# mic-rud/Learned-Compression-of-Point-Cloud-Geometry-and-Attributes

Hardware: AMD Instinct MI355X
Metric: encode+decode Mpoints/sec (higher is better)
Workload: dtype f32

## Files before the change

include/pcc_hip.h:

```cpp
#ifndef PCC_HIP_H
#define PCC_HIP_H

#include <stdint.h>

#ifdef __cplusplus
extern "C" {
#endif

#define PCC_OK 0
#define PCC_ERR_ARG (-1)
#define PCC_ERR_HIP (-2)
#define PCC_ERR_UNSUPPORTED (-3)
#define PCC_ERR_DATA (-4)

#define PCC_ACT_NONE 0
#define PCC_ACT_RELU 1
#define PCC_ACT_LEAKY_RELU 2

int pcc_version(void);
const char* pcc_last_error(void);
int pcc_device_count(void);
int pcc_device_name(int dev, char* out, int out_len);

int64_t pcc_hash_capacity(int64_t n);
// ... 37 lines not shown
                   int32_t sign, int32_t* nbr, uint32_t* row_mask, int64_t* pair_count,
                   void* stream);

int pcc_pair_count(const uint32_t* row_mask, int64_t n_out, int64_t* pair_count, void* stream);

int64_t pcc_order_scratch_bytes(int64_t n);
int pcc_order_rows_by_mask(const uint32_t* row_mask, const int32_t* coords, int64_t n,
                           int32_t block_log2, int32_t tensor_stride, int32_t* order, uint32_t* group_mask32,
                           void* scratch, int64_t scratch_bytes, void* stream);
int pcc_permute_map_rows(const int32_t* nbr, const int32_t* order, int64_t n, int32_t K, int32_t* nbr_sorted, void* stream);

int64_t pcc_small_map_max(void);
int32_t pcc_small_paths(int32_t mask);
int pcc_small_kernel_map(const int32_t* out_coords, int64_t n_out, const uint64_t* in_keys, const int32_t* in_vals, int64_t in_cap,
                         int32_t ksize, int32_t step, int32_t sign, int32_t* nbr, uint32_t* row_mask, int32_t* order,
                         uint32_t* group_mask32, void* scratch, int64_t scratch_bytes, void* stream);

int64_t pcc_conv_packed_elems(int32_t K, int32_t cin, int32_t cout);
int pcc_conv_pack_weights(const float* w, int32_t K, int32_t cin, int32_t cout, float* w_packed,
                          void* stream);
int pcc_conv_fwd(const float* fin, int64_t n_in, int32_t cin, const float* w, const float* w_packed,
                 const float* bias, const int32_t* nbr, const int32_t* order,
                 const uint32_t* group_mask32, int32_t K, float* fout, int64_t n_out, int32_t cout,
                 int32_t act, const float* film, const float* residual, void* stream);

int64_t pcc_conv_small_max(int64_t workgroups);

int pcc_conv_kernel_name(int32_t mode, int64_t n_in, int32_t cin, int32_t cout, int64_t n_out, int32_t K, int32_t has_nbr,
                         char* buf, int32_t len);

int64_t pcc_conv_packed_elems_bf16(int32_t K, int32_t cin, int32_t cout);
int pcc_conv_pack_weights_bf16(const float* w, int32_t K, int32_t cin, int32_t cout, uint16_t* w_packed, void* stream);
int pcc_conv_fwd_bf16(const uint16_t* fin, int64_t n_in, int32_t cin, const uint16_t* w_packed, const float* bias,
                      const int32_t* nbr, const int32_t* order, const uint32_t* group_mask32, int32_t K, float* fout,
                      int64_t n_out, int32_t cout, int32_t act, const float* film, const float* residual, void* stream);

int pcc_epilogue_fwd(const float* c, const float* film, const float* residual, int64_t n, int32_t channels, int32_t act,
                     float* out, void* stream);
int pcc_epilogue_bwd(const float* dout, const float* c, const float* film, int64_t n, int32_t channels, int32_t act,
                     float* dc, float* dfilm, void* stream);

int64_t pcc_cast_colsum_scratch_elems(int32_t channels);
int pcc_cast_colsum(const float* x, int64_t n, int32_t channels, uint16_t* out_bf16, float* colsum, float* scratch,
                    int64_t scratch_elems, void* stream);

int64_t pcc_conv_packed_elems_x3(int32_t K, int32_t cin, int32_t cout);
int pcc_conv_pack_weights_x3(const float* w, int32_t K, int32_t cin, int32_t cout, uint16_t* w_packed, void* stream);
int pcc_conv_fwd_x3(const float* fin, int64_t n_in, int32_t cin, const uint16_t* w_packed, const float* bias,
                    const int32_t* nbr, const int32_t* order, const uint32_t* group_mask32, int32_t K, float* fout,
                    int64_t n_out, int32_t cout, int32_t act, const float* film, const float* residual, void* stream);

int pcc_im2col_thin(const float* fin, int32_t cin, const int32_t* nbr, int64_t n_out, int32_t K, float* out, int32_t k2,
                    void* stream);

int pcc_gather_sum_fwd(const float* scores, int32_t ld, const int32_t* nbr, int32_t K, int32_t cout,
                       const float* bias, float* out, int64_t n_out, int32_t act, void* stream);

int pcc_gather_rows(const float* src, int32_t c, const int32_t* idx, int64_t n, float* out,
                    int32_t accumulate, void* stream);

int pcc_scatter_rows(const float* src, int32_t c, const int32_t* idx, int64_t n, float* out,
                     void* stream);
int pcc_scatter_add_rows(const float* src, int32_t c, const int32_t* idx, int64_t n, float* out,
                         void* stream);

int pcc_compact_rows(const uint8_t* mask, int64_t n, const int32_t* coords, int32_t* out_coords,
                     const float* feats, int32_t c, float* out_feats, int32_t* new_index,
                     int32_t* scratch, int64_t* out_count, void* stream);

int64_t pcc_topk_state_elems(int32_t nbatch);
int pcc_topk_mask(const float* logits, int32_t ld, const int32_t* coords, int64_t n, int32_t nbatch,
                  const int32_t* k, uint8_t* mask, int32_t* state, void* stream);

int pcc_count_per_batch(const int32_t* coords, int64_t n, int32_t nbatch, int32_t* counts, void* stream);

int64_t pcc_sort_scratch_bytes(int64_t n);
int pcc_sort_coords(const int32_t* coords, int64_t n, int32_t* perm, void* scratch,
                    int64_t scratch_bytes, void* stream);

int pcc_kernel_map_transpose(const int32_t* nbr, int64_t n_out, int32_t K, int64_t n_in, int32_t* nbr_t,
                             uint32_t* row_mask_t, void* stream);
int64_t pcc_conv_wgrad_scratch_elems(int32_t K, int32_t cin, int32_t cout);
int pcc_conv_wgrad(const float* fin, int64_t n_in, int32_t cin, const float* dy, int64_t n_out, int32_t cout,
                   const int32_t* nbr, const int32_t* order, const uint32_t* group_mask32, int32_t K, float* dw,
                   float* scratch, int64_t scratch_elems, void* stream);
int pcc_conv_wgrad_kernel_name(int32_t bf16, int32_t K, int32_t cin, int32_t cout, int64_t n_out, char* buf, int32_t len,
                               int32_t* split, int32_t* partials);
int pcc_conv_wgrad_bf16(const uint16_t* fin, int64_t n_in, int32_t cin, const uint16_t* dy, int64_t n_out, int32_t cout,
                        const int32_t* nbr, const int32_t* order, const uint32_t* group_mask32, int32_t K, float* dw,
                        float* scratch, int64_t scratch_elems, void* stream);

int pcc_chconv(const float* x, int64_t n, int32_t c, const int32_t* coords, const uint64_t* keys, const int32_t* vals,
               int64_t cap, int32_t tensor_stride, int32_t ksize, const float* w, int32_t w_channels, int32_t flip,
               float* y, void* stream);

int64_t pcc_octree_scratch_bytes(int64_t n);
int pcc_octree_occupancy(const int32_t* coords, int64_t n, int32_t stride, const int32_t* origin,
                         int32_t depth, uint8_t* occupancy, int32_t* level_counts, void* scratch,
                         int64_t scratch_bytes, void* stream);
int pcc_octree_expand(const uint8_t* occupancy, const int64_t* level_counts, int32_t depth,
                      int32_t stride, const int32_t* origin, int32_t batch, int64_t n_points,
                      int32_t* coords_out, void* scratch, int64_t scratch_bytes, void* stream);

int pcc_nn_search(const int32_t* query, int64_t nq, const uint64_t* keys, const int32_t* vals, int64_t cap,
                  int32_t tensor_stride, const double* target_rgb, int32_t max_radius, int32_t* nn_idx, int64_t* nn_d2,
                  int32_t* tie_count, double* tie_rgb, void* stream);
// ... 92 lines not shown
```

learned-compression-of-point-cloud-geometry-and-attributes_amd/_build.py:

```python
import os
import subprocess

_HERE = os.path.dirname(os.path.abspath(__file__))
SO_PATH = os.path.join(_HERE, "libpcc_hip.so")

NO_SCRATCH = {
    "conv": ("conv_small_kernel", "conv_mfma_buf_kernel", "conv_mfma_kernel"),
    "rans_lanes": ("rans_lanes_encode_kernel", "rans_lanes_pack_kernel", "rans_lanes_decode_kernel"),
    "chconv": ("chconv_kernel",),
    "augment": ("jitter_partial_kernel", "jitter_mean_kernel", "jitter_apply_kernel", "first_rows_clear_kernel",
                "first_rows_insert_kernel", "first_rows_flag_kernel", "first_rows_finalize_kernel"),
    "normals": ("estimate_normals_kernel",),
    "voxelize": ("first_rows_clear_kernel", "first_rows_insert_kernel", "first_rows_flag_kernel", "first_rows_finalize_kernel",
                 "voxelize_accumulate_kernel"),
    "raht": ("raht_plan_kernel", "raht_step_kernel", "raht_fold_kernel"),
}


def build(force=False):
    args = ["make", "-s", "-C", os.path.join(_HERE, "csrc"), "-j4"]
    if force:
        subprocess.check_call(args + ["clean"])
    subprocess.check_call(args)
    for stem, kernels in NO_SCRATCH.items():
        check_kernel_resources(os.path.join(_HERE, "build", stem + ".resources.txt"), kernels)
    check_small_kernel_lds_reads()
    return SO_PATH


def check_small_kernel_lds_reads(obj=None):
    import glob
    import shutil
    objdump = "/opt/rocm/lib/llvm/bin/llvm-objdump"
    obj = obj or os.path.join(_HERE, "build", "conv.o")
    if not os.path.exists(objdump) or not os.path.exists(obj):
        raise RuntimeError(f"cannot lint conv_small_kernel: {objdump} or {obj} is missing")
    tmp = os.path.join(_HERE, "build", "_lint")
    shutil.rmtree(tmp, ignore_errors=True)
    os.makedirs(tmp)
    local = os.path.join(tmp, "conv.o")
    shutil.copy(obj, local)
    subprocess.run([objdump, "--offloading", local], check=True, capture_output=True, cwd=tmp)
    cos = [f for f in glob.glob(local + ".*") if "amdgcn" in f]
    if not cos:
        raise RuntimeError("cannot lint conv_small_kernel: no device code object in build/conv.o")
    dis = subprocess.run([objdump, "-d", cos[0]], check=True, capture_output=True, text=True).stdout
    shutil.rmtree(tmp, ignore_errors=True)
    return lint_lds_reads(dis)


def lint_lds_reads(dis, kernel="conv_small_kernel"):
    import re

    def regs(operand):
        m = re.fullmatch(r"v\[(\d+):(\d+)\]", operand)
        if m:
            return set(range(int(m.group(1)), int(m.group(2)) + 1))
        m = re.fullmatch(r"v(\d+)", operand)
        return {int(m.group(1))} if m else set()

# ... 64 lines not shown
```

learned-compression-of-point-cloud-geometry-and-attributes_amd/csrc/conv.hip:

```cpp
#include <stdlib.h>

#include <type_traits>

#include "common.h"

namespace pcc {

typedef float f32x2 __attribute__((ext_vector_type(2)));
typedef float f32x4 __attribute__((ext_vector_type(4)));
typedef __bf16 bf16x8 __attribute__((ext_vector_type(8)));

struct ConvArgs {
    const float* fin;
    const float* w;
    const float* wp;
    const float* bias;
    const int32_t* nbr;
    const int32_t* order;
    const uint32_t* gmask;
    float* fout;
    const float* film;
    const float* residual;
    int64_t n_in, n_out;
    int cin, cout, coutp, K, act;
// ... 768 lines not shown
        for (int j = 0; j < CPT; ++j) acc[j] = 0.0f;
        for (int k0 = 0; k0 < K; k0 += 9) {
            int idx[9];
#pragma unroll
            for (int u = 0; u < 9; ++u) idx[u] = (k0 + u < K) ? (a.nbr ? a.nbr[row * K + k0 + u] : (int)row) : -1;
            float in[9][CIN];
#pragma unroll
            for (int u = 0; u < 9; ++u) {
                const int64_t src = idx[u] >= 0 ? idx[u] : 0;
#pragma unroll
                for (int ci = 0; ci < CIN; ++ci) in[u][ci] = a.fin[src * CIN + ci];
            }
#pragma unroll
            for (int u = 0; u < 9; ++u) {
                if (idx[u] < 0) continue;
                const float* wk = smem + ((k0 + u) * CIN) * cout + co;
#pragma unroll
                for (int ci = 0; ci < CIN; ++ci)
#pragma unroll
                    for (int j = 0; j < CPT; ++j) acc[j] = fmaf(in[u][ci], wk[ci * cout + j], acc[j]);
            }
        }
#pragma unroll
        for (int j = 0; j < CPT; ++j) conv_store(a, row, co + j, acc[j], conv_bias(a, co + j));
    }
}

__global__ __launch_bounds__(256) void im2col_thin_kernel(const float* __restrict__ fin, int cin, const int32_t* __restrict__ nbr,
                                                          int64_t n_out, int K, float* __restrict__ out, int k2) {
    const int q = k2 >> 2;
    const int64_t total = n_out * q;
    const int kc = K * cin;
    for (int64_t e = (int64_t)blockIdx.x * 256 + threadIdx.x; e < total; e += (int64_t)gridDim.x * 256) {
        const int64_t row = e / q;
        const int c0 = (int)(e - row * q) * 4;
        f32x4 v;
#pragma unroll
        for (int s = 0; s < 4; ++s) {
            const int c = c0 + s;
            const int s8 = c & 7;
            const int logical = (c & ~7) + ((s8 & 3) << 1 | (s8 >> 2));
            float x = 0.0f;
            if (logical < kc) {
                const int k = logical / cin, ci = logical - k * cin;
                const int idx = nbr[row * K + k];
                if (idx >= 0) x = fin[(int64_t)idx * cin + ci];
            }
            v[s] = x;
        }
        *reinterpret_cast<f32x4*>(out + row * k2 + c0) = v;
    }
}

__global__ __launch_bounds__(256) void gather_sum_kernel(const float* __restrict__ scores, int ld,
                                                         const int32_t* __restrict__ nbr, int K, int cout,
                                                         const float* __restrict__ bias, float* __restrict__ out,
                                                         int64_t n_out, int act) {
    const int64_t total = n_out * cout;
    for (int64_t e = (int64_t)blockIdx.x * 256 + threadIdx.x; e < total; e += (int64_t)gridDim.x * 256) {
        const int64_t row = e / cout;
        const int c = (int)(e - row * cout);
        float acc = 0.0f;
        for (int k = 0; k < K; ++k) {
            const int idx = nbr[row * K + k];
            if (idx >= 0) acc += scores[(int64_t)idx * ld + k * cout + c];
        }
        out[e] = apply_act(acc + (bias ? bias[c] : 0.0f), act);
    }
}

template <int COUT>
__global__ __launch_bounds__(256) void gather_sum27_kernel(const float* __restrict__ scores, int ld,
                                                           const int32_t* __restrict__ nbr, const float* __restrict__ bias,
                                                           float* __restrict__ out, int64_t n_out, int act) {
    __shared__ __attribute__((aligned(16))) int32_t idx_s[256 * 27];
    const int64_t row0 = (int64_t)blockIdx.x * 256;
    const int64_t rows = (n_out - row0 < 256) ? (n_out - row0) : 256;
    const int64_t words = rows * 27;
    const int32_t* src = nbr + row0 * 27;
    for (int64_t w = 4 * (int64_t)threadIdx.x; w < words; w += 1024) {
        if (w + 4 <= words) {
            *reinterpret_cast<int4*>(idx_s + w) = *reinterpret_cast<const int4*>(src + w);
        } else {
            for (int64_t u = w; u < words; ++u) idx_s[u] = src[u];
        }
    }
    __syncthreads();
    if ((int64_t)threadIdx.x >= rows) return;
    const int32_t* mine = idx_s + threadIdx.x * 27;
    float acc[COUT];
#pragma unroll
    for (int c = 0; c < COUT; ++c) acc[c] = 0.0f;
#pragma unroll
    for (int k0 = 0; k0 < 27; k0 += 9) {
        int idx[9];
        float v[9][COUT];
#pragma unroll
        for (int u = 0; u < 9; ++u) idx[u] = mine[k0 + u];
#pragma unroll
        for (int u = 0; u < 9; ++u) {
            const float* sp = scores + (int64_t)(idx[u] >= 0 ? idx[u] : 0) * ld + (k0 + u) * COUT;
#pragma unroll
            for (int c = 0; c < COUT; ++c) v[u][c] = sp[c];
        }
#pragma unroll
        for (int u = 0; u < 9; ++u)
            if (idx[u] >= 0) {
#pragma unroll
                for (int c = 0; c < COUT; ++c) acc[c] += v[u][c];
            }
    }
    float* o = out + (row0 + threadIdx.x) * COUT;
#pragma unroll
    for (int c = 0; c < COUT; ++c) o[c] = apply_act(acc[c] + (bias ? bias[c] : 0.0f), act);
}

enum ConvMode { CONV_F32 = 0, CONV_BF16 = 1, CONV_X3 = 2 };
static const char* const CONV_ENTRY[] = {"pcc_conv_fwd", "pcc_conv_fwd_bf16", "pcc_conv_fwd_x3"};
static const char* const CONV_TAG[] = {"", "[bf16]", "[x3]"};

enum ConvFamily { FAM_THIN, FAM_SMALL, FAM_BUF, FAM_GLOBAL };

struct ConvPlan {
    ConvFamily family;
    int bm, bn, wm, wn;
    int cch;
    int sc, ns;
    int cpt;
};

constexpr int64_t FILL_WGS = 768;
constexpr int64_t ROW32_MAX_WGS = 3000;

static inline int round_up32(int v) { return (v + 31) / 32 * 32; }

static bool fits_buffer_path(const ConvArgs& a) {
    const uint64_t lim = BUF_OOB;
    return (uint64_t)a.n_in * a.cin * 4 <= lim && (uint64_t)a.n_out * a.K * 4 <= lim && (uint64_t)a.K * a.cin * a.coutp * 4 <= lim;
}

static int conv_path() {
    static int path = -1;
    if (path < 0) { const char* e = getenv("PCC_CONV_PATH"); path = (e && e[0] == 'g') ? 1 : 0; }
    return path;
}

static int64_t g_small_max = -1;
static int64_t small_max_value() {
    if (g_small_max < 0) { const char* e = getenv("PCC_CONV_SMALL_MAX"); g_small_max = e ? atoll(e) : 640; }
    return g_small_max;
}

static bool thin_cin(int cin) {
    for (int c : {1, 2, 3, 4, 6, 8, 12, 16, 24})
        if (cin == c) return true;
    return false;
}

static int check_shape(const ConvArgs& a, ConvMode mode, const char* who) {
    PCC_REQUIRE(a.K >= 1 && a.K <= 27, "%s: K=%d out of range", who, a.K);
    if (mode == CONV_F32) PCC_REQUIRE(a.cin % 32 != 0 || a.cin <= 256, "%s: MFMA path supports cin <= 256 (got %d)", who, a.cin);
    if (mode == CONV_BF16) PCC_REQUIRE(a.cin % 64 == 0 && a.cin <= 256, "%s: cin must be a multiple of 64 up to 256 (got %d)", who, a.cin);
    if (mode == CONV_X3) PCC_REQUIRE(a.cin % 32 == 0 && a.cin <= 256, "%s: cin must be a multiple of 32 up to 256 (got %d)", who, a.cin);
    PCC_REQUIRE(a.nbr != nullptr || (a.K == 1 && a.n_in == a.n_out), "%s: nbr == NULL needs K == 1 and n_in == n_out", who);
    return PCC_OK;
}

static int plan_conv(const ConvArgs& a, ConvMode mode, ConvPlan& p, const char* who) {
    p = ConvPlan{};
    if (mode == CONV_F32 && a.cin % 32 != 0) {
        if (!thin_cin(a.cin)) {
            pcc::set_error("%s: unsupported cin=%d (need a multiple of 32 or one of 1,2,3,4,6,8,12,16,24)", who, a.cin);
            return PCC_ERR_UNSUPPORTED;
        }
        const size_t lds = (size_t)a.K * a.cin * a.cout * sizeof(float);
        PCC_REQUIRE(lds <= 160 * 1024, "conv(thin): weights %zu B exceed the 160 KB of LDS (cin=%d cout=%d K=%d)", lds, a.cin, a.cout, a.K);
        p.family = FAM_THIN;
        p.cpt = (a.cout % 8 == 0) ? 8 : (a.cout % 4 == 0) ? 4 : (a.cout % 2 == 0) ? 2 : 1;
        return PCC_OK;
    }
    const bool wide = a.coutp % 128 == 0;
    p.family = FAM_BUF;
    p.cch = a.cin / (mode == CONV_BF16 ? 64 : 32);
    if (mode == CONV_F32) {
        const bool buffer = conv_path() == 0 && fits_buffer_path(a);
        const int64_t wgs32 = ((a.n_out + 31) / 32) * (a.coutp / 32);
        if (a.nbr && buffer && wgs32 <= small_max_value() * (wide ? 1 : 2)) {
            p.family = FAM_SMALL;
            p.sc = (p.cch % 4 == 0 && wgs32 <= 256) ? 4 : p.cch % 2 == 0 ? 2 : 1;
            p.ns = p.sc == 1 ? 8 : 3;
            return PCC_OK;
        }
        if (!buffer) p.family = FAM_GLOBAL;
    } else if (mode == CONV_BF16) {
        PCC_REQUIRE((uint64_t)a.n_in * a.cin * 2 <= BUF_OOB && (uint64_t)a.n_out * a.K * 4 <= BUF_OOB,
                    "%s: operands of 4 GiB and more are not supported", who);
    } else {
        PCC_REQUIRE((uint64_t)a.n_in * a.cin * 4 <= BUF_OOB && (uint64_t)a.n_out * a.K * 4 <= BUF_OOB &&
                    (uint64_t)a.K * a.cin * a.coutp * 6 <= BUF_OOB, "%s: operands of 4 GiB and more are not supported", who);
    }
    const int64_t wgs128 = ((a.n_out + 63) / 64) * (a.coutp / 128);
    auto tile = [&](int bm, int bn, int wm, int wn) { p.bm = bm; p.bn = bn; p.wm = wm; p.wn = wn; return PCC_OK; };
    if (wide && wgs128 < FILL_WGS) return tile(64, 64, 2, 2);
    if (wide && mode == CONV_F32 && wgs128 < ROW32_MAX_WGS) return tile(32, 128, 1, 4);
    if (wide) return tile(64, 128, 2, 2);
    if (a.coutp % 64 == 0) return mode == CONV_X3 ? tile(64, 64, 2, 2) : tile(128, 64, 2, 2);
    if (mode != CONV_X3) return tile(128, 32, 4, 1);
    pcc::set_error("%s: cout=%d not supported (output width rounded up to 32 must be a multiple of 64)", who, a.cout);
    return PCC_ERR_UNSUPPORTED;
}

template <auto KERN>
static int launch(int64_t blocks, int threads, size_t lds, size_t lds_limit, const ConvArgs& a, hipStream_t st) {
    static bool limit_set = false;
    if (lds_limit && !limit_set) {
        PCC_CHECK_HIP(hipFuncSetAttribute(reinterpret_cast<const void*>(KERN), hipFuncAttributeMaxDynamicSharedMemorySize, (int)lds_limit));
        limit_set = true;
    }
    PCC_REQUIRE(blocks < (1ll << 31), "conv: grid too large");
    hipLaunchKernelGGL(KERN, dim3((unsigned)blocks), dim3(threads), lds, st, a);
    PCC_LAUNCH_CHECK();
    return PCC_OK;
}

template <ConvMode M, int BM, int BN, int WM, int WN, int CCH>
static int launch_buf(int64_t blocks, const ConvArgs& a, hipStream_t st) {
    constexpr bool BF16 = M == CONV_BF16, X3 = M == CONV_X3;
    if constexpr (BF16 && CCH > 4) {
        return PCC_ERR_UNSUPPORTED;
    } else {
        constexpr int lds = conv_lds_bytes<BM, BN, X3>();
        return a.nbr ? launch<conv_mfma_buf_kernel<BM, BN, WM, WN, CCH, true, BF16, X3>>(blocks, 256, lds, lds, a, st)
                     : launch<conv_mfma_buf_kernel<BM, BN, WM, WN, CCH, false, BF16, X3>>(blocks, 256, lds, lds, a, st);
    }
}

template <ConvMode M, int BM, int BN, int WM, int WN>
static int launch_mfma(const ConvPlan& p, const ConvArgs& a, hipStream_t st) {
    const int64_t blocks = (a.n_out + BM - 1) / BM * (a.coutp / BN);
    if constexpr (M == CONV_F32) {
        if (p.family == FAM_GLOBAL) {
            constexpr int lds = conv_lds_bytes<BM, BN>();
            return a.nbr ? launch<conv_mfma_kernel<BM, BN, WM, WN, true>>(blocks, 256, lds, lds, a, st)
                         : launch<conv_mfma_kernel<BM, BN, WM, WN, false>>(blocks, 256, lds, lds, a, st);
        }
    }
    switch (p.cch) {
        case 1: return launch_buf<M, BM, BN, WM, WN, 1>(blocks, a, st);
        case 2: return launch_buf<M, BM, BN, WM, WN, 2>(blocks, a, st);
        case 3: return launch_buf<M, BM, BN, WM, WN, 3>(blocks, a, st);
        case 4: return launch_buf<M, BM, BN, WM, WN, 4>(blocks, a, st);
        case 5: return launch_buf<M, BM, BN, WM, WN, 5>(blocks, a, st);
        case 6: return launch_buf<M, BM, BN, WM, WN, 6>(blocks, a, st);
        case 7: return launch_buf<M, BM, BN, WM, WN, 7>(blocks, a, st);
        case 8: return launch_buf<M, BM, BN, WM, WN, 8>(blocks, a, st);
        default: return PCC_ERR_UNSUPPORTED;
    }
}

template <ConvMode M>
static int launch_tile(const ConvPlan& p, const ConvArgs& a, hipStream_t st) {
    if (p.bm == 64 && p.bn == 64) return launch_mfma<M, 64, 64, 2, 2>(p, a, st);
    if (p.bm == 64 && p.bn == 128) return launch_mfma<M, 64, 128, 2, 2>(p, a, st);
    if constexpr (M == CONV_F32)
        if (p.bm == 32) return launch_mfma<M, 32, 128, 1, 4>(p, a, st);
    if constexpr (M != CONV_X3) {
        if (p.bn == 64) return launch_mfma<M, 128, 64, 2, 2>(p, a, st);
        if (p.bn == 32) return launch_mfma<M, 128, 32, 4, 1>(p, a, st);
    }
    return PCC_ERR_UNSUPPORTED;
}

template <int SC, int NS>
static int launch_small(const ConvArgs& a, hipStream_t st) {
    constexpr int lds = conv_small_lds_bytes<SC, NS>();
    return launch<conv_small_kernel<SC, NS>>(((a.n_out + 31) / 32) * (a.coutp / 32), 512, lds, lds, a, st);
}

template <int CIN>
static int launch_thin(const ConvPlan& p, const ConvArgs& a, hipStream_t st) {
    const size_t lds = (size_t)a.K * CIN * a.cout * sizeof(float);
    const unsigned nb = blocks_for(a.n_out * (a.cout / p.cpt), 256, lds >= 4096 ? 2048u : (1u << 20));
    const size_t limit = lds > 64 * 1024 ? 160 * 1024 : 0;
    if (p.cpt == 8) return launch<conv_thin_kernel<CIN, 8>>(nb, 256, lds, limit, a, st);
    if (p.cpt == 4) return launch<conv_thin_kernel<CIN, 4>>(nb, 256, lds, limit, a, st);
    if (p.cpt == 2) return launch<conv_thin_kernel<CIN, 2>>(nb, 256, lds, limit, a, st);
    return launch<conv_thin_kernel<CIN, 1>>(nb, 256, lds, limit, a, st);
}

static int launch_thin_cin(const ConvPlan& p, const ConvArgs& a, hipStream_t st) {
    switch (a.cin) {
        case 1: return launch_thin<1>(p, a, st);
        case 2: return launch_thin<2>(p, a, st);
        case 3: return launch_thin<3>(p, a, st);
        case 4: return launch_thin<4>(p, a, st);
        case 6: return launch_thin<6>(p, a, st);
        case 8: return launch_thin<8>(p, a, st);
        case 12: return launch_thin<12>(p, a, st);
        case 16: return launch_thin<16>(p, a, st);
        case 24: return launch_thin<24>(p, a, st);
        default: return PCC_ERR_UNSUPPORTED;
    }
}

static int conv_fwd(ConvMode mode, const ConvArgs& a, void* stream) {
    const char* who = CONV_ENTRY[mode];
    int rc = check_shape(a, mode, who);
    if (rc != PCC_OK) return rc;
    PCC_REQUIRE(a.act >= 0 && a.act <= 2, "%s: bad activation %d", who, a.act);
    if (mode == CONV_F32 && a.n_out <= 0) return PCC_OK;
    if (mode != CONV_F32 || a.cin % 32 == 0) {
        PCC_REQUIRE(a.wp != nullptr, "%s: MFMA path (cin=%d) needs packed weights", who, a.cin);
        PCC_REQUIRE(((reinterpret_cast<uintptr_t>(a.fin) | reinterpret_cast<uintptr_t>(a.wp)) & 15) == 0,
                    "%s: fin and w_packed must be 16-byte aligned (16-byte LDS-DMA loads)", who);
    } else {
        PCC_REQUIRE(a.w != nullptr, "%s: thin path (cin=%d) needs raw weights", who, a.cin);
    }
    if (a.n_out <= 0) return PCC_OK;
    ConvPlan p;
    if ((rc = plan_conv(a, mode, p, who)) != PCC_OK) return rc;
    hipStream_t st = as_stream(stream);
    switch (p.family) {
// ... 24 lines not shown
using namespace pcc;

extern "C" {

int64_t pcc_conv_packed_elems(int32_t K, int32_t cin, int32_t cout) {
    return (int64_t)K * round_up32(cin) * round_up32(cout);
}

int pcc_conv_pack_weights(const float* w, int32_t K, int32_t cin, int32_t cout, float* w_packed, void* stream) {
    return pack_weights("pcc_conv_pack_weights", pack_weights_kernel, 32, w, K, cin, cout, w_packed, stream);
}

int64_t pcc_conv_packed_elems_bf16(int32_t K, int32_t cin, int32_t cout) {
    return (int64_t)K * ((cin + 63) / 64 * 64) * round_up32(cout);
}

int pcc_conv_pack_weights_bf16(const float* w, int32_t K, int32_t cin, int32_t cout, uint16_t* w_packed, void* stream) {
    return pack_weights("pcc_conv_pack_weights_bf16", pack_weights_bf16_kernel, 64, w, K, cin, cout,
                        reinterpret_cast<__bf16*>(w_packed), stream);
}

int pcc_conv_fwd_bf16(const uint16_t* fin, int64_t n_in, int32_t cin, const uint16_t* w_packed, const float* bias, const int32_t* nbr,
                      const int32_t* order, const uint32_t* group_mask32, int32_t K, float* fout, int64_t n_out, int32_t cout,
                      int32_t act, const float* film, const float* residual, void* stream) {
    return conv_fwd(CONV_BF16, {reinterpret_cast<const float*>(fin), nullptr, reinterpret_cast<const float*>(w_packed), bias, nbr, order,
                                group_mask32, fout, film, residual, n_in, n_out, cin, cout, round_up32(cout), K, act}, stream);
}

int64_t pcc_conv_packed_elems_x3(int32_t K, int32_t cin, int32_t cout) {
    return (int64_t)K * round_up32(cin) * round_up32(cout) * 3;
}

int pcc_conv_pack_weights_x3(const float* w, int32_t K, int32_t cin, int32_t cout, uint16_t* w_packed, void* stream) {
    return pack_weights("pcc_conv_pack_weights_x3", pack_weights_x3_kernel, 32, w, K, cin, cout, w_packed, stream);
}

int pcc_conv_fwd_x3(const float* fin, int64_t n_in, int32_t cin, const uint16_t* w_packed, const float* bias, const int32_t* nbr,
                    const int32_t* order, const uint32_t* group_mask32, int32_t K, float* fout, int64_t n_out, int32_t cout,
                    int32_t act, const float* film, const float* residual, void* stream) {
    return conv_fwd(CONV_X3, {fin, nullptr, reinterpret_cast<const float*>(w_packed), bias, nbr, order, group_mask32, fout, film,
                              residual, n_in, n_out, cin, cout, round_up32(cout), K, act}, stream);
}

int pcc_im2col_thin(const float* fin, int32_t cin, const int32_t* nbr, int64_t n_out, int32_t K, float* out, int32_t k2,
                    void* stream) {
    PCC_REQUIRE(K >= 1 && K <= 27 && cin >= 1 && cin <= 16, "pcc_im2col_thin: bad shape (K=%d cin=%d)", K, cin);
    PCC_REQUIRE(k2 % 32 == 0 && k2 >= K * cin, "pcc_im2col_thin: row length %d must be a multiple of 32 and >= K * cin = %d", k2, K * cin);
    PCC_REQUIRE(nbr != nullptr && (reinterpret_cast<uintptr_t>(out) & 15) == 0, "pcc_im2col_thin: nbr required, out 16-byte aligned");
    if (n_out <= 0) return PCC_OK;
    hipLaunchKernelGGL(im2col_thin_kernel, dim3(blocks_for(n_out * (k2 / 4), 256, 1 << 20)), dim3(256), 0, as_stream(stream), fin, cin, nbr,
                       n_out, K, out, k2);
    PCC_LAUNCH_CHECK();
    return PCC_OK;
}

int pcc_gather_sum_fwd(const float* scores, int32_t ld, const int32_t* nbr, int32_t K, int32_t cout, const float* bias,
                       float* out, int64_t n_out, int32_t act, void* stream) {
    PCC_REQUIRE(K >= 1 && K <= 27 && cout >= 1 && ld >= K * cout, "pcc_gather_sum_fwd: bad shape (K=%d cout=%d ld=%d)", K, cout, ld);
    PCC_REQUIRE(nbr != nullptr, "pcc_gather_sum_fwd: neighbour table required");
    PCC_REQUIRE(act >= 0 && act <= 2, "pcc_gather_sum_fwd: bad activation %d", act);
    if (n_out <= 0) return PCC_OK;
    const unsigned nb27 = blocks_for(n_out, 256);
    const bool al16 = (reinterpret_cast<uintptr_t>(nbr) & 15) == 0;
#define PCC_GS27(C)                                                                                                    \
    hipLaunchKernelGGL(gather_sum27_kernel<C>, dim3(nb27), dim3(256), 0, as_stream(stream), scores, ld, nbr, bias, out, n_out, act)
    if (K == 27 && al16 && cout == 1) PCC_GS27(1);
    else if (K == 27 && al16 && cout == 2) PCC_GS27(2);
    else if (K == 27 && al16 && cout == 3) PCC_GS27(3);
    else if (K == 27 && al16 && cout == 4) PCC_GS27(4);
    else
#undef PCC_GS27
        hipLaunchKernelGGL(gather_sum_kernel, dim3(blocks_for(n_out * cout, 256, 1 << 20)), dim3(256), 0, as_stream(stream),
                           scores, ld, nbr, K, cout, bias, out, n_out, act);
    PCC_LAUNCH_CHECK();
    return PCC_OK;
}

int64_t pcc_conv_small_max(int64_t workgroups) {
    const int64_t before = small_max_value();
    if (workgroups >= 0) g_small_max = workgroups;
    return before;
}

int pcc_conv_fwd(const float* fin, int64_t n_in, int32_t cin, const float* w, const float* w_packed, const float* bias,
                 const int32_t* nbr, const int32_t* order, const uint32_t* group_mask32, int32_t K, float* fout,
                 int64_t n_out, int32_t cout, int32_t act, const float* film, const float* residual, void* stream) {
    return conv_fwd(CONV_F32, {fin, w, w_packed, bias, nbr, order, group_mask32, fout, film, residual, n_in, n_out, cin, cout,
                               round_up32(cout), K, act}, stream);
}

int pcc_conv_kernel_name(int32_t mode, int64_t n_in, int32_t cin, int32_t cout, int64_t n_out, int32_t K, int32_t has_nbr,
                         char* buf, int32_t len) {
    PCC_REQUIRE(mode >= CONV_F32 && mode <= CONV_X3, "pcc_conv_kernel_name: bad mode %d", mode);
    static const int32_t any_map = 0;
    ConvArgs a = {};
    a.nbr = has_nbr ? &any_map : nullptr;
    a.n_in = n_in; a.n_out = n_out; a.cin = cin; a.cout = cout; a.coutp = round_up32(cout); a.K = K;
    const ConvMode m = ConvMode(mode);
    ConvPlan p;
    if (check_shape(a, m, CONV_ENTRY[m]) != PCC_OK || plan_conv(a, m, p, CONV_ENTRY[m]) != PCC_OK) return PCC_ERR_UNSUPPORTED;
    if (buf == nullptr) return PCC_OK;
    const char* tf = has_nbr ? "true" : "false";
    int n;
    if (p.family == FAM_THIN) n = snprintf(buf, len, "conv_thin_kernel<%d, %d>", cin, p.cpt);
    else if (p.family == FAM_SMALL) n = snprintf(buf, len, "conv_small_kernel<%d, %d>", p.sc, p.ns);
    else if (p.family == FAM_GLOBAL) n = snprintf(buf, len, "conv_mfma_kernel<%d, %d, %d, %d, %s>", p.bm, p.bn, p.wm, p.wn, tf);
    else n = snprintf(buf, len, "conv_mfma_buf_kernel%s<%d, %d, %d, %d, %d, %s>", CONV_TAG[m], p.bm, p.bn, p.wm, p.wn, p.cch, tf);
    PCC_REQUIRE(n < len, "pcc_conv_kernel_name: %d bytes do not hold the name", len);
    return PCC_OK;
}

}
```

learned-compression-of-point-cloud-geometry-and-attributes_amd/sparse.py:

```python
import ctypes
import functools
import math
import weakref

import os

import torch
import torch.nn as nn

from . import _lib, _threads
from ._lib import PCC, check, ptr

ACT_NONE, ACT_RELU, ACT_LRELU = PCC.ACT_NONE, PCC.ACT_RELU, PCC.ACT_LEAKY_RELU


def _require_cuda(t):
    if not t.is_cuda:
        raise RuntimeError("libpcc_hip operators need tensors on an MI355X device (got a CPU tensor); "
                           "there is no CPU fallback")


COORD_PROFILER = None


def _cp_begin():
    if COORD_PROFILER is None:
        return None
    ev = torch.cuda.Event(enable_timing=True)
    ev.record()
    return ev


def _cp_end(ev0, name, rows, alg_bytes):
    if ev0 is None or COORD_PROFILER is None:
        return
    ev1 = torch.cuda.Event(enable_timing=True)
    ev1.record()
    main = torch.cuda.current_stream() == torch.cuda.default_stream()
    COORD_PROFILER.append((name, int(rows), alg_bytes, ev0, ev1, main))


def _as_int_coords(coords):
    if coords.dtype.is_floating_point:
        coords = torch.floor(coords)
    return coords.to(torch.int32).contiguous()


def _host_count():
    st = _threads.current()
    if st.count is None:
        buf = torch.zeros(1, dtype=torch.int64, pin_memory=True)
        st.count = (buf, buf.numpy())
    st.count[1][0] = COUNT_ARMED
    return st.count


_SMALL_MAP_MAX = None


def _small_map_max():
    global _SMALL_MAP_MAX
    if _SMALL_MAP_MAX is None:
        _SMALL_MAP_MAX = int(_lib.lib().pcc_small_map_max())
    return _SMALL_MAP_MAX


def set_small_map_max(rows):
    global _SMALL_MAP_MAX
    was = _small_map_max()
    _SMALL_MAP_MAX = min(int(rows), int(_lib.lib().pcc_small_map_max())) if rows else 0
    return was


def set_small_paths(mask):
    return int(_lib.lib().pcc_small_paths(int(mask)))


class CoordinateRangeError(ValueError):
    """a coordinate outside the voxel key's range (|c| <= PCC_COORD_LIMIT, 0 <= batch index <= PCC_BATCH_LIMIT: include/pcc_hip.h)"""


COUNT_ARMED, COUNT_ERR_RANGE = -1, PCC.COUNT_ERR_RANGE


def _read_count(word, device):
    import time
    deadline = time.perf_counter() + 2e-3
    while word[0] == COUNT_ARMED:
        if time.perf_counter() > deadline:
            torch.cuda.current_stream(device).synchronize()
            break
        time.sleep(0)
    n = int(word[0])
    if n == COUNT_ERR_RANGE:
        raise CoordinateRangeError(f"libpcc_hip: a voxel coordinate is outside the supported range (|c| <= {PCC.COORD_LIMIT}, batch "
                                   f"index <= {PCC.BATCH_LIMIT}): the 18-bit fields of the voxel key would alias — translate the cloud "
                                   "towards the origin or re-voxelise it")
    if n < 0:
        raise RuntimeError("libpcc_hip: the row count was never written (kernel failure?)")
    return n


def _set_buffers(m, dev):
    L = _lib.lib()
    cap = L.pcc_hash_capacity(m)
    return (torch.empty(cap, dtype=torch.int64, device=dev), torch.empty(cap, dtype=torch.int32, device=dev), cap,
            torch.empty(L.pcc_scan_scratch_elems(m), dtype=torch.int32, device=dev))


class PairCount:

    def __init__(self, row_mask):
        self._mask, self._val = row_mask, None

    def item(self):
        if self._val is None:
            out = torch.empty(1, dtype=torch.int64, device=self._mask.device)
            check(_lib.lib().pcc_pair_count(ptr(self._mask), self._mask.shape[0], ptr(out), _lib.stream()))
            self._val = int(out.item())
        return self._val

    __int__ = item

    def __float__(self):
        return float(self.item())


def _same_map(kept, out_map, self_map):
# ... 407 lines not shown
    out = torch.empty((n_out, cout), dtype=torch.float32, device=x_feats.device)
    mode = launch_mode(INFER_BF16, INFER_X3, n_in, cin, cout, n_out, K, nbr is not None) if INFER_BF16 or INFER_X3 else MODE_F32
    prof = PROFILER
    timed = prof is not None and n_out >= PROFILER_MIN_ROWS
    if not timed and mode == MODE_F32:
        check(L.pcc_conv_fwd(x_feats.data_ptr(), n_in, cin, w.data_ptr(), None if wp is None else wp.data_ptr(),
                             None if bias is None else bias.data_ptr(), None if nbr is None else nbr.data_ptr(),
                             None if order is None else order.data_ptr(), None if gmask is None else gmask.data_ptr(), K,
                             out.data_ptr(), n_out, cout, act, None if film is None else film.data_ptr(),
                             None if residual is None else residual.data_ptr(), _lib.stream()))
        if prof is not None:
            prof.append((("conv", mode, n_in, K, nbr is not None), cin, cout, pairs if pairs is not None else n_out, n_out,
                         None, None, gmask))
        return out
    ev0 = _prof_begin(timed)
    launch_conv(mode, x_feats, w, layer.packed(mode, out_channels), bias, nbr, order, gmask, out, act, film, residual)
    _prof_end(ev0, ("conv", mode, n_in, K, nbr is not None), cin, cout, pairs if pairs is not None else n_out, n_out, gmask)
    return out


def profiled_name(entry):
    name, cin, cout, _, n_out = entry[:5]
    if isinstance(name, tuple):
        _, mode, n_in, K, has_nbr = name
        return conv_kernel_name(mode, n_in, cin, cout, n_out, K, has_nbr)
    return name


def _prof_begin(timed=True):
    if PROFILER is None or not timed:
        return None
    ev = torch.cuda.Event(enable_timing=True)
    ev.record()
    return ev


def _prof_end(ev0, name, cin, cout, pairs, n_out, gmask=None):
    if PROFILER is None:
        return
    ev1 = None
    if ev0 is not None:
        ev1 = torch.cuda.Event(enable_timing=True)
        ev1.record()
    PROFILER.append((name, cin, cout, pairs, n_out, ev0, ev1, gmask))


_MFMA_VISIT = (0, 4, 1, 5, 2, 6, 3, 7)


def _thin_im2col_forward(x_feats, in_map, out_map, layer, ksize, transposed, act, film, residual, out_channels):
    L = _lib.lib()
    w2p, bias, k2, cout = layer.im2col_weights(out_channels)
    nbr, _, pairs = in_map.kernel_map(out_map, ksize, transposed)
    n_out, K, cin = out_map.n, ksize ** 3, x_feats.shape[1]
    dev = x_feats.device
    x2 = torch.empty((n_out, k2), dtype=torch.float32, device=dev)
    out = torch.empty((n_out, cout), dtype=torch.float32, device=dev)
    ev0 = _prof_begin()
    ev = _cp_begin()
    check(L.pcc_im2col_thin(ptr(x_feats), cin, ptr(nbr), n_out, K, ptr(x2), k2, _lib.stream()))
    _cp_end(ev, "im2col_thin", n_out, lambda: 4 * K * n_out + 4 * cin * int(pairs) + 4 * k2 * n_out)
    check(L.pcc_conv_fwd(ptr(x2), n_out, k2, None, ptr(w2p), ptr(bias), None, None, None, 1, ptr(out), n_out, cout, act, ptr(film),
                         ptr(residual), _lib.stream()))
    _prof_end(ev0, f"thin_im2col<{cin}>", cin, cout, pairs, n_out)
    return out


def _narrow_head_forward(x_feats, in_map, out_map, layer, ksize, transposed, act, out_channels):
    L = _lib.lib()
    w_r, wp_r, bias, K, cout = layer.narrow_weights(out_channels)
    n_in, cin = x_feats.shape
    n_out = out_map.n
    nbr, _, pairs = in_map.kernel_map(out_map, ksize, transposed)
    ld = K * cout
    scores = torch.empty((n_in, ld), dtype=torch.float32, device=x_feats.device)
    out = torch.empty((n_out, cout), dtype=torch.float32, device=x_feats.device)
    ev0 = _prof_begin()
    check(L.pcc_conv_fwd(ptr(x_feats), n_in, cin, ptr(w_r), ptr(wp_r), None, None, None, None, 1, ptr(scores), n_in, ld,
                         ACT_NONE, None, None, _lib.stream()))
    ev = _cp_begin()
    check(L.pcc_gather_sum_fwd(ptr(scores), ld, ptr(nbr), K, cout, ptr(bias), ptr(out), n_out, act, _lib.stream()))
    _cp_end(ev, "gather_sum", n_out, lambda: 4 * K * n_out + 4 * cout * int(pairs) + 4 * cout * n_out)
    _prof_end(ev0, f"narrow_head<{cin}>", cin, cout, pairs, n_out)
    return out


def set_conv_small_max(workgroups):
    return int(_lib.lib().pcc_conv_small_max(int(workgroups)))


NARROW_HEAD_MAX_COUT = 4

CHECK_EXPECTED_COUNTS = os.environ.get("PCC_CHECK_COUNTS", "0") == "1"
ORDER_BLOCK_LOG2 = int(os.environ.get("PCC_ORDER_BLOCK_LOG2", "-1"))

INFER_BF16 = os.environ.get("PCC_INFER_BF16", "0") == "1"


def set_infer_bf16(enabled):
    global INFER_BF16
    INFER_BF16 = bool(enabled)


INFER_X3 = os.environ.get("PCC_INFER_X3", "0") == "1"


def set_infer_x3(enabled):
    global INFER_X3
    INFER_X3 = bool(enabled)


GATE_LOG = None


PROFILER = None
PROFILER_MIN_ROWS = 65536


MODE_F32, MODE_BF16, MODE_X3 = 0, 1, 2


def conv_kernel_name(mode, n_in, cin, cout, n_out, K, has_nbr):
    buf = ctypes.create_string_buffer(128)
    check(_lib.lib().pcc_conv_kernel_name(mode, n_in, cin, cout, n_out, K, int(has_nbr), buf, len(buf)))
    return buf.value.decode()


def launch_mode(bf16, x3, n_in, cin, cout, n_out, K, has_nbr):
    if bf16 and _plan_takes(MODE_BF16, n_in, cin, cout, n_out, K, has_nbr):
        return MODE_BF16
    if x3 and _plan_takes(MODE_X3, n_in, cin, cout, n_out, K, has_nbr):
        return MODE_X3
    return MODE_F32


@functools.lru_cache(maxsize=4096)
def _plan_takes(mode, n_in, cin, cout, n_out, K, has_nbr):
    return _lib.lib().pcc_conv_kernel_name(mode, n_in, cin, cout, n_out, K, int(has_nbr), None, 0) == 0


def launch_conv(mode, feats, w, wp, bias, nbr, order, gmask, out, act=ACT_NONE, film=None, residual=None):
    L = _lib.lib()
    K, cin, cout = w.shape
    n_in, n_out = feats.shape[0], out.shape[0]
    if mode == MODE_BF16:
        check(L.pcc_conv_fwd_bf16(ptr(feats.to(torch.bfloat16)), n_in, cin, ptr(wp), ptr(bias), ptr(nbr), ptr(order), ptr(gmask), K,
                                  ptr(out), n_out, cout, act, ptr(film), ptr(residual), _lib.stream()))
    elif mode == MODE_X3:
        check(L.pcc_conv_fwd_x3(ptr(feats), n_in, cin, ptr(wp), ptr(bias), ptr(nbr), ptr(order), ptr(gmask), K, ptr(out), n_out,
                                cout, act, ptr(film), ptr(residual), _lib.stream()))
    else:
        check(L.pcc_conv_fwd(ptr(feats), n_in, cin, ptr(w), ptr(wp), ptr(bias), ptr(nbr), ptr(order), ptr(gmask), K, ptr(out),
                             n_out, cout, act, ptr(film), ptr(residual), _lib.stream()))


def pack_weights(w, mode=MODE_F32):
    K, cin, cout = w.shape
    if mode == MODE_F32 and cin % 32:
        return None
    L = _lib.lib()
    suffix = ("", "_bf16", "_x3")[mode]
    wp = torch.empty(getattr(L, "pcc_conv_packed_elems" + suffix)(K, cin, cout),
                     dtype=torch.float32 if mode == MODE_F32 else torch.bfloat16, device=w.device)
    check(getattr(L, "pcc_conv_pack_weights" + suffix)(ptr(w), K, cin, cout, ptr(wp), _lib.stream()))
    return wp


def _cached_weights(slot, with_bias=True):
    def wrap(f):
        @functools.wraps(f)
        def cached(self, out_channels=None):
            params = self._parameters
            kernel, bias = params["kernel"], params.get("bias") if with_bias else None
            key = (kernel._version, kernel.data_ptr(), out_channels, None if bias is None else (bias._version, bias.data_ptr()))
            hit = self._packed.get(slot)
            if hit is not None and hit[0] == key:
                return hit[1]
            res = f(self, out_channels)
            self._packed[slot] = (key, res)
            return res
        return cached
    return wrap


class _ConvBase(nn.Module):
    transposed = False
    generative = False

    def __init__(self, in_channels, out_channels, kernel_size=-1, stride=1, dilation=1, bias=False, dimension=3):
        super().__init__()
        assert dimension == 3 and dilation == 1
# ... 186 lines not shown
```

Before: 9.032.

## Fuse thin-channel im2col gather into the MFMA conv kernel

Adds conv_thin_gather_kernel, which gathers neighbour rows for thin-input convolutions (cin 1/2/4/8) straight into LDS A tiles with buffer loads, and feeds them to the existing MFMA step. This drops the separate im2col pass and its materialised (n_out, k2) intermediate buffer. The Python thin-im2col path uses it by default when the plan supports it, and falls back to the old path otherwise. The cost is an extra neighbour-index table in LDS and irregular gathers inside the GEMM loop, which may lower occupancy or overlap compared with the plain buffered kernel.

```diff
diff --git a/include/pcc_hip.h b/include/pcc_hip.h
--- a/include/pcc_hip.h
+++ b/include/pcc_hip.h
@@ -113,6 +113,10 @@
 
 int pcc_im2col_thin(const float* fin, int32_t cin, const int32_t* nbr, int64_t n_out, int32_t K, float* out, int32_t k2,
                     void* stream);
+
+int pcc_conv_fwd_thin_gather(const float* fin, int64_t n_in, int32_t cin, const int32_t* nbr, int32_t K, const float* w2p,
+                             int32_t k2, const float* bias, float* out, int64_t n_out, int32_t cout, int32_t act,
+                             const float* film, const float* residual, void* stream);
 
 int pcc_gather_sum_fwd(const float* scores, int32_t ld, const int32_t* nbr, int32_t K, int32_t cout,
                        const float* bias, float* out, int64_t n_out, int32_t act, void* stream);
diff --git a/learned-compression-of-point-cloud-geometry-and-attributes_amd/_build.py b/learned-compression-of-point-cloud-geometry-and-attributes_amd/_build.py
--- a/learned-compression-of-point-cloud-geometry-and-attributes_amd/_build.py
+++ b/learned-compression-of-point-cloud-geometry-and-attributes_amd/_build.py
@@ -5,7 +5,7 @@
 SO_PATH = os.path.join(_HERE, "libpcc_hip.so")
 
 NO_SCRATCH = {
-    "conv": ("conv_small_kernel", "conv_mfma_buf_kernel", "conv_mfma_kernel"),
+    "conv": ("conv_small_kernel", "conv_mfma_buf_kernel", "conv_mfma_kernel", "conv_thin_gather_kernel"),
     "rans_lanes": ("rans_lanes_encode_kernel", "rans_lanes_pack_kernel", "rans_lanes_decode_kernel"),
     "chconv": ("chconv_kernel",),
     "augment": ("jitter_partial_kernel", "jitter_mean_kernel", "jitter_apply_kernel", "first_rows_clear_kernel",
diff --git a/learned-compression-of-point-cloud-geometry-and-attributes_amd/csrc/conv.hip b/learned-compression-of-point-cloud-geometry-and-attributes_amd/csrc/conv.hip
--- a/learned-compression-of-point-cloud-geometry-and-attributes_amd/csrc/conv.hip
+++ b/learned-compression-of-point-cloud-geometry-and-attributes_amd/csrc/conv.hip
@@ -844,6 +844,154 @@
     }
 }
 
+template <int BM, int BN>
+constexpr int conv_thin_gather_lds_bytes(int K) { return conv_lds_bytes<BM, BN>() / 2 + BM * K * (int)sizeof(uint32_t); }
+
+template <int BM, int BN, int WAVES_M, int WAVES_N, int CCH>
+__global__ __launch_bounds__(256) void conv_thin_gather_kernel(const ConvArgs a) {
+#if defined(__HIP_DEVICE_COMPILE__)
+    constexpr int WM = BM / WAVES_M, WN = BN / WAVES_N;
+    constexpr int MT = WM / 32, NT = WN / 32;
+    constexpr int A_ELEMS = BM * 32;
+    constexpr int W_ELEMS = 8 * BN * 4;
+    constexpr int W_LOADS = (8 * BN) / 256;
+    static_assert(WAVES_M * WAVES_N == 4 && MT >= 1 && MT <= 2 && NT >= 1 && W_LOADS >= 1, "bad tiling");
+
+    extern __shared__ __attribute__((aligned(16))) float smem[];
+    float* As = smem;
+    float* Ws = smem + A_ELEMS;
+    uint32_t* Is = reinterpret_cast<uint32_t*>(smem + A_ELEMS + W_ELEMS);
+
+    const int t = threadIdx.x;
+    const int lane = t & 63, wid = t >> 6;
+    const int r = lane & 31, h = lane >> 5;
+    const int wrow = (wid / WAVES_N) * WM, wcol = (wid % WAVES_N) * WN;
+
+    const int ntiles_n = a.coutp / BN;
+    const int64_t tile = blockIdx.x / ntiles_n;
+    const int nt = blockIdx.x - (int)(tile * ntiles_n);
+    const int64_t row0 = tile * BM;
+    const int K = a.K;
+
+    __amdgpu_buffer_rsrc_t rsrc_a = __builtin_amdgcn_make_buffer_rsrc(
+        const_cast<float*>(a.fin), 0, (int)(uint32_t)(a.n_in * a.cin * 4), BUF_FLAGS);
+    __amdgpu_buffer_rsrc_t rsrc_w = __builtin_amdgcn_make_buffer_rsrc(
+        const_cast<float*>(a.wp), 0, (int)((uint32_t)(32 * CCH) * a.coutp * 4), BUF_FLAGS);
+
+    {
+        constexpr int IDX_LOADS = (BM * 27 + 255) / 256;
+        const int64_t first = row0 * K, end = a.n_out * K;
+        const uint32_t row_bytes = (uint32_t)a.cin * 4;
+        int idx[IDX_LOADS];
+#pragma unroll
+        for (int j = 0; j < IDX_LOADS; ++j) {
+            const int e = t + 256 * j;
+            idx[j] = (e < BM * K && first + e < end) ? a.nbr[first + e] : -1;
+        }
+#pragma unroll
+        for (int j = 0; j < IDX_LOADS; ++j) {
+            const int e = t + 256 * j;
+            if (e < BM * K) Is[e] = idx[j] >= 0 ? (uint32_t)idx[j] * row_bytes : BUF_OOB;
+        }
+    }
+
+    const int wave_u = __builtin_amdgcn_readfirstlane(wid);
+    uint32_t w_voff[W_LOADS];
+#pragma unroll
+    for (int j = 0; j < W_LOADS; ++j) {
+        const int f = t + 256 * j;
+        const int g = f / BN, col = f - g * BN;
+        w_voff[j] = (uint32_t)((g * a.coutp + nt * BN + col) * 16);
+    }
+    const uint32_t w_cstride = 8u * a.coutp * 16;
+    constexpr int ITEMS = (BM * 4 + 255) / 256;
+    int irow[ITEMS], ig[ITEMS], a_put[ITEMS][2];
+    bool ival[ITEMS];
+#pragma unroll
+    for (int i = 0; i < ITEMS; ++i) {
+        const int item = t + 256 * i;
+        const int row = item % BM, g = item / BM;
+        const int sw = (row >> 1) & 7;
+        ival[i] = g < 4;
+        irow[i] = row * K;
+        ig[i] = g;
+        a_put[i][0] = row * 32 + ((2 * g) ^ sw) * 4;
+        a_put[i][1] = row * 32 + ((2 * g + 1) ^ sw) * 4;
+    }
+
+    float stage[ITEMS][8];
+    auto gather_cin = [&](auto cc, auto cinc) {
+        constexpr int c = decltype(cc)::value;
+        constexpr int CIN = decltype(cinc)::value;
+        constexpr int LC = CIN == 1 ? 0 : CIN == 2 ? 1 : CIN == 4 ? 2 : 3;
+#pragma unroll
+        for (int i = 0; i < ITEMS; ++i) {
+            const int k0 = (32 * c + 8 * ig[i]) >> LC;
+#pragma unroll
+            for (int j = 0; j < (CIN == 8 ? 1 : 8 / CIN); ++j) {
+                const uint32_t off = (ival[i] && k0 + j < K) ? Is[irow[i] + k0 + j] : BUF_OOB;
+                if constexpr (CIN == 1) {
+                    stage[i][j] = __builtin_bit_cast(float, __builtin_amdgcn_raw_buffer_load_b32(rsrc_a, off, 0, 0));
+                } else if constexpr (CIN == 2) {
+                    const f32x2 v = __builtin_bit_cast(f32x2, __builtin_amdgcn_raw_buffer_load_b64(rsrc_a, off, 0, 0));
+                    stage[i][2 * j] = v[0];
+                    stage[i][2 * j + 1] = v[1];
+                } else {
+#pragma unroll
+                    for (int q = 0; q < CIN / 4; ++q) {
+                        const f32x4 v = __builtin_bit_cast(f32x4, __builtin_amdgcn_raw_buffer_load_b128(rsrc_a, off + 16 * q, 0, 0));
+#pragma unroll
+                        for (int e = 0; e < 4; ++e) stage[i][4 * (CIN == 8 ? q : j) + e] = v[e];
+                    }
+                }
+            }
+        }
+    };
+    auto gather = [&](auto cc) {
+        if (a.cin == 2) gather_cin(cc, std::integral_constant<int, 2>{});
+        else if (a.cin == 4) gather_cin(cc, std::integral_constant<int, 4>{});
+        else if (a.cin == 8) gather_cin(cc, std::integral_constant<int, 8>{});
+        else gather_cin(cc, std::integral_constant<int, 1>{});
+    };
+    auto put = [&]() {
+#pragma unroll
+        for (int i = 0; i < ITEMS; ++i) {
+            if (!ival[i]) continue;
+            *reinterpret_cast<f32x4*>(As + a_put[i][0]) = f32x4{stage[i][0], stage[i][2], stage[i][4], stage[i][6]};
+            *reinterpret_cast<f32x4*>(As + a_put[i][1]) = f32x4{stage[i][1], stage[i][3], stage[i][5], stage[i][7]};
+        }
+    };
+    auto dma_w = [&](auto cc) {
+        constexpr int c = decltype(cc)::value;
+#pragma unroll
+        for (int j = 0; j < W_LOADS; ++j)
+            __builtin_amdgcn_raw_ptr_buffer_load_lds(rsrc_w, (lds_ptr_t)(Ws + (wave_u * 64 + 256 * j) * 4), 16,
+                                                     w_voff[j], (uint32_t)c * w_cstride, 0, 0);
+    };
+
+    uint32_t a_addr[4];
+#pragma unroll
+    for (int kk = 0; kk < 4; ++kk) a_addr[kk] = a_frag_offset(wrow + r, h, kk);
+    const uint32_t w_addr = (uint32_t)((A_ELEMS + (h * BN + wcol + r) * 4) * 4);
+
+    f32x16 acc[MT][NT] = {};
+
+    dma_w(std::integral_constant<int, 0>{});
+    __syncthreads();
+    static_for<0, CCH>([&](auto cc) {
+        constexpr int c = decltype(cc)::value;
+        if constexpr (c > 0) dma_w(cc);
+        gather(cc);
+        put();
+        __syncthreads();
+        mfma_step<(1u << MT) - 1u, BN, false>(acc, a_addr, w_addr);
+        if constexpr (c + 1 < CCH) __syncthreads();
+    });
+
+    conv_store_tiles(a, acc, row0 + wrow, nt * BN + wcol + r, h);
+#endif
+}
+
 __global__ __launch_bounds__(256) void gather_sum_kernel(const float* __restrict__ scores, int ld,
                                                          const int32_t* __restrict__ nbr, int K, int cout,
                                                          const float* __restrict__ bias, float* __restrict__ out,
@@ -910,6 +1058,7 @@
 enum ConvMode { CONV_F32 = 0, CONV_BF16 = 1, CONV_X3 = 2 };
 static const char* const CONV_ENTRY[] = {"pcc_conv_fwd", "pcc_conv_fwd_bf16", "pcc_conv_fwd_x3"};
 static const char* const CONV_TAG[] = {"", "[bf16]", "[x3]"};
+constexpr int CONV_THIN_GATHER = 3;
 
 enum ConvFamily { FAM_THIN, FAM_SMALL, FAM_BUF, FAM_GLOBAL };
 
@@ -1002,6 +1151,23 @@
     return PCC_ERR_UNSUPPORTED;
 }
 
+static int plan_thin_gather(const ConvArgs& a, ConvPlan& p, bool& fused, const char* who) {
+    PCC_REQUIRE(a.K >= 1 && a.K <= 27, "%s: K=%d out of range", who, a.K);
+    PCC_REQUIRE(a.cin == 1 || a.cin == 2 || a.cin == 4 || a.cin == 8, "%s: cin=%d (need 1, 2, 4 or 8)", who, a.cin);
+    PCC_REQUIRE(a.nbr != nullptr, "%s: neighbour table required", who);
+    ConvArgs g = a;
+    g.cin = round_up32(a.K * a.cin);
+    g.K = 1;
+    g.nbr = nullptr;
+    g.n_in = a.n_out;
+    const int rc = plan_conv(g, CONV_F32, p, who);
+    if (rc != PCC_OK) return rc;
+    const uint64_t lim = BUF_OOB;
+    fused = p.family == FAM_BUF && (p.cch == 1 || p.cch == 2 || p.cch == 4 || p.cch == 7) &&
+            (uint64_t)a.n_in * a.cin * 4 <= lim && (uint64_t)a.n_out * a.K * 4 <= lim;
+    return PCC_OK;
+}
+
 template <auto KERN>
 static int launch(int64_t blocks, int threads, size_t lds, size_t lds_limit, const ConvArgs& a, hipStream_t st) {
     static bool limit_set = false;
@@ -1060,6 +1226,28 @@
         if (p.bn == 64) return launch_mfma<M, 128, 64, 2, 2>(p, a, st);
         if (p.bn == 32) return launch_mfma<M, 128, 32, 4, 1>(p, a, st);
     }
+    return PCC_ERR_UNSUPPORTED;
+}
+
+template <int BM, int BN, int WM, int WN>
+static int launch_thin_gather_cch(const ConvPlan& p, const ConvArgs& a, hipStream_t st) {
+    const int64_t blocks = (a.n_out + BM - 1) / BM * (a.coutp / BN);
+    const size_t lds = conv_thin_gather_lds_bytes<BM, BN>(a.K), limit = conv_thin_gather_lds_bytes<BM, BN>(27);
+    switch (p.cch) {
+        case 1: return launch<conv_thin_gather_kernel<BM, BN, WM, WN, 1>>(blocks, 256, lds, limit, a, st);
+        case 2: return launch<conv_thin_gather_kernel<BM, BN, WM, WN, 2>>(blocks, 256, lds, limit, a, st);
+        case 4: return launch<conv_thin_gather_kernel<BM, BN, WM, WN, 4>>(blocks, 256, lds, limit, a, st);
+        case 7: return launch<conv_thin_gather_kernel<BM, BN, WM, WN, 7>>(blocks, 256, lds, limit, a, st);
+        default: return PCC_ERR_UNSUPPORTED;
+    }
+}
+
+static int launch_thin_gather(const ConvPlan& p, const ConvArgs& a, hipStream_t st) {
+    if (p.bm == 64 && p.bn == 64) return launch_thin_gather_cch<64, 64, 2, 2>(p, a, st);
+    if (p.bm == 64 && p.bn == 128) return launch_thin_gather_cch<64, 128, 2, 2>(p, a, st);
+    if (p.bm == 32) return launch_thin_gather_cch<32, 128, 1, 4>(p, a, st);
+    if (p.bn == 64) return launch_thin_gather_cch<128, 64, 2, 2>(p, a, st);
+    if (p.bn == 32) return launch_thin_gather_cch<128, 32, 4, 1>(p, a, st);
     return PCC_ERR_UNSUPPORTED;
 }
 
@@ -1190,6 +1378,28 @@
                        n_out, K, out, k2);
     PCC_LAUNCH_CHECK();
     return PCC_OK;
+}
+
+int pcc_conv_fwd_thin_gather(const float* fin, int64_t n_in, int32_t cin, const int32_t* nbr, int32_t K, const float* w2p, int32_t k2,
+                             const float* bias, float* out, int64_t n_out, int32_t cout, int32_t act, const float* film,
+                             const float* residual, void* stream) {
+    const char* who = "pcc_conv_fwd_thin_gather";
+    const ConvArgs a = {fin, nullptr, w2p, bias, nbr, nullptr, nullptr, out, film, residual, n_in, n_out, cin, cout, round_up32(cout), K, act};
+    ConvPlan p;
+    bool fused = false;
+    const int rc = plan_thin_gather(a, p, fused, who);
+    if (rc != PCC_OK) return rc;
+    PCC_REQUIRE(k2 == round_up32(K * cin), "%s: row length %d must be K * cin = %d rounded up to 32", who, k2, K * cin);
+    PCC_REQUIRE(act >= 0 && act <= 2, "%s: bad activation %d", who, act);
+    PCC_REQUIRE(w2p != nullptr && ((reinterpret_cast<uintptr_t>(w2p) | reinterpret_cast<uintptr_t>(fin)) & 15) == 0,
+                "%s: w2p required; fin and w2p 16-byte aligned (a row's channels are one load; LDS-DMA loads)", who);
+    PCC_REQUIRE(n_in >= 1 || n_out <= 0, "%s: no input rows", who);
+    if (n_out <= 0) return PCC_OK;
+    if (!fused) {
+        pcc::set_error("%s: this shape runs as pcc_im2col_thin + pcc_conv_fwd (pcc_conv_kernel_name, mode 3, tells)", who);
+        return PCC_ERR_UNSUPPORTED;
+    }
+    return launch_thin_gather(p, a, as_stream(stream));
 }
 
 int pcc_gather_sum_fwd(const float* scores, int32_t ld, const int32_t* nbr, int32_t K, int32_t cout, const float* bias,
@@ -1229,18 +1439,27 @@
 
 int pcc_conv_kernel_name(int32_t mode, int64_t n_in, int32_t cin, int32_t cout, int64_t n_out, int32_t K, int32_t has_nbr,
                          char* buf, int32_t len) {
-    PCC_REQUIRE(mode >= CONV_F32 && mode <= CONV_X3, "pcc_conv_kernel_name: bad mode %d", mode);
+    PCC_REQUIRE(mode >= CONV_F32 && mode <= CONV_THIN_GATHER, "pcc_conv_kernel_name: bad mode %d", mode);
     static const int32_t any_map = 0;
     ConvArgs a = {};
     a.nbr = has_nbr ? &any_map : nullptr;
     a.n_in = n_in; a.n_out = n_out; a.cin = cin; a.cout = cout; a.coutp = round_up32(cout); a.K = K;
-    const ConvMode m = ConvMode(mode);
+    ConvMode m = ConvMode(mode);
     ConvPlan p;
-    if (check_shape(a, m, CONV_ENTRY[m]) != PCC_OK || plan_conv(a, m, p, CONV_ENTRY[m]) != PCC_OK) return PCC_ERR_UNSUPPORTED;
+    bool fused = false;
+    if (mode == CONV_THIN_GATHER) {
+        if (plan_thin_gather(a, p, fused, "pcc_conv_fwd_thin_gather") != PCC_OK) return PCC_ERR_UNSUPPORTED;
+        m = CONV_F32;
+        has_nbr = 0;
+        cin = round_up32(K * cin);
+    } else if (check_shape(a, m, CONV_ENTRY[m]) != PCC_OK || plan_conv(a, m, p, CONV_ENTRY[m]) != PCC_OK) {
+        return PCC_ERR_UNSUPPORTED;
+    }
     if (buf == nullptr) return PCC_OK;
     const char* tf = has_nbr ? "true" : "false";
     int n;
-    if (p.family == FAM_THIN) n = snprintf(buf, len, "conv_thin_kernel<%d, %d>", cin, p.cpt);
+    if (fused) n = snprintf(buf, len, "conv_thin_gather_kernel<%d, %d, %d, %d, %d>", p.bm, p.bn, p.wm, p.wn, p.cch);
+    else if (p.family == FAM_THIN) n = snprintf(buf, len, "conv_thin_kernel<%d, %d>", cin, p.cpt);
     else if (p.family == FAM_SMALL) n = snprintf(buf, len, "conv_small_kernel<%d, %d>", p.sc, p.ns);
     else if (p.family == FAM_GLOBAL) n = snprintf(buf, len, "conv_mfma_kernel<%d, %d, %d, %d, %s>", p.bm, p.bn, p.wm, p.wn, tf);
     else n = snprintf(buf, len, "conv_mfma_buf_kernel%s<%d, %d, %d, %d, %d, %s>", CONV_TAG[m], p.bm, p.bn, p.wm, p.wn, p.cch, tf);
diff --git a/learned-compression-of-point-cloud-geometry-and-attributes_amd/sparse.py b/learned-compression-of-point-cloud-geometry-and-attributes_amd/sparse.py
--- a/learned-compression-of-point-cloud-geometry-and-attributes_amd/sparse.py
+++ b/learned-compression-of-point-cloud-geometry-and-attributes_amd/sparse.py
@@ -74,6 +74,15 @@
 
 def set_small_paths(mask):
     return int(_lib.lib().pcc_small_paths(int(mask)))
+
+
+_THIN_GATHER = os.environ.get("PCC_THIN_GATHER", "1") != "0"
+
+
+def set_thin_gather(on):
+    global _THIN_GATHER
+    was, _THIN_GATHER = _THIN_GATHER, bool(on)
+    return was
 
 
 class CoordinateRangeError(ValueError):
@@ -587,11 +596,16 @@
     L = _lib.lib()
     w2p, bias, k2, cout = layer.im2col_weights(out_channels)
     nbr, _, pairs = in_map.kernel_map(out_map, ksize, transposed)
-    n_out, K, cin = out_map.n, ksize ** 3, x_feats.shape[1]
+    n_out, K, (n_in, cin) = out_map.n, ksize ** 3, x_feats.shape
     dev = x_feats.device
-    x2 = torch.empty((n_out, k2), dtype=torch.float32, device=dev)
     out = torch.empty((n_out, cout), dtype=torch.float32, device=dev)
     ev0 = _prof_begin()
+    if _THIN_GATHER and not (INFER_BF16 or INFER_X3) and _thin_gather_takes(n_in, cin, cout, n_out, K):
+        check(L.pcc_conv_fwd_thin_gather(ptr(x_feats), n_in, cin, ptr(nbr), K, ptr(w2p), k2, ptr(bias), ptr(out), n_out, cout, act,
+                                         ptr(film), ptr(residual), _lib.stream()))
+        _prof_end(ev0, f"thin_im2col<{cin}>", cin, cout, pairs, n_out)
+        return out
+    x2 = torch.empty((n_out, k2), dtype=torch.float32, device=dev)
     ev = _cp_begin()
     check(L.pcc_im2col_thin(ptr(x_feats), cin, ptr(nbr), n_out, K, ptr(x2), k2, _lib.stream()))
     _cp_end(ev, "im2col_thin", n_out, lambda: 4 * K * n_out + 4 * cin * int(pairs) + 4 * k2 * n_out)
@@ -672,6 +686,14 @@
 @functools.lru_cache(maxsize=4096)
 def _plan_takes(mode, n_in, cin, cout, n_out, K, has_nbr):
     return _lib.lib().pcc_conv_kernel_name(mode, n_in, cin, cout, n_out, K, int(has_nbr), None, 0) == 0
+
+
+MODE_THIN_GATHER = 3
+
+
+@functools.lru_cache(maxsize=4096)
+def _thin_gather_takes(n_in, cin, cout, n_out, K):
+    return conv_kernel_name(MODE_THIN_GATHER, n_in, cin, cout, n_out, K, True).startswith("conv_thin_gather_kernel")
 
 
 def launch_conv(mode, feats, w, wp, bias, nbr, order, gmask, out, act=ACT_NONE, film=None, residual=None):
```

After: 8.887. 0.984x the previous value.
